# GuixingLin/akka-allreduce

Measured on AMD Instinct MI355X. Metric: allreduce algbw (GB/s) on 256 MB fp32 buffer at 1/2/4/8 MI355X, higher is better.
Workload: dtype fp32

## Files before the change

### akka_allreduce_amd/_build.py

```python
from __future__ import annotations

import concurrent.futures as cf
import glob
import os
import shlex
import subprocess
import sys
import sysconfig

ROOT = os.path.dirname(os.path.dirname(os.path.abspath(__file__)))
CSRC = os.path.join(ROOT, "csrc")
BUILD = os.path.join(ROOT, "build", "native")
PKG = os.path.join(ROOT, "akka_allreduce_amd")
ROCM = os.environ.get("ROCM_PATH", "/opt/rocm")
ARCH = os.environ.get("AKKA_OFFLOAD_ARCH", "gfx950")

HOST_SOURCES = [
    "engine/host_device.cpp",
    "engine/racecheck.cpp",
    "engine/dataplane.cpp",
    "engine/engine.cpp",
    "transport/sim_p2p.cpp",
    "transport/stream_link.cpp",
    "transport/reactive_link.cpp",
    "transport/rccl_p2p.cpp",
    "transport/ipc_lane.cpp",
    "transport/ipc_p2p.cpp",
    "transport/onesided.cpp",
    "transport/link_probe.cpp",
    "kernels/hip_device.cpp",
    "runtime/watchdog.cpp",
    "bindings/bindings.cpp",
    "bindings/bind_onesided.cpp",
    "bindings/bind_probe.cpp",
]
HIP_SOURCES = [
    "kernels/reduce.hip",
    "kernels/counts.hip",
    "kernels/optim.hip",
    "kernels/pack_bf16.hip",
    "kernels/colsum.hip",
    "kernels/xent.hip",
    "kernels/ipc.hip",
    "kernels/onesided.hip",
    "kernels/probe.hip",
]


def ext_path() -> str:
    return os.path.join(PKG, "_native" + sysconfig.get_config_var("EXT_SUFFIX"))


def _torch_lib() -> str:
    import importlib.util

    spec = importlib.util.find_spec("torch")
    if spec is None or not spec.origin:
        raise RuntimeError("torch is required to locate the HIP runtime / RCCL it ships")
    return os.path.join(os.path.dirname(spec.origin), "lib")


def _headers() -> list[str]:
    return sorted(glob.glob(os.path.join(CSRC, "**", "*.h"), recursive=True))


def _stale(obj: str, src: str, headers: list[str]) -> bool:
    if not os.path.exists(obj):
        return True
    t = os.path.getmtime(obj)
    return os.path.getmtime(src) > t or any(os.path.getmtime(h) > t for h in headers)


def source_hash(root: str | None = None) -> str | None:
    import hashlib

    csrc = os.path.join(root or ROOT, "csrc")
    files = [os.path.join(csrc, r) for r in HOST_SOURCES + HIP_SOURCES]
    files += sorted(glob.glob(os.path.join(csrc, "**", "*.h"), recursive=True))
    if not all(os.path.exists(f) for f in files[: len(HOST_SOURCES) + len(HIP_SOURCES)]):
        return None
    h = hashlib.sha256(ARCH.encode())
    for f in files:
        if not os.path.exists(f):
            continue
        h.update(os.path.relpath(f, csrc).encode() + b"\0")
        with open(f, "rb") as fh:
            h.update(fh.read())
        h.update(b"\0")
    return h.hexdigest()


def hash_path(ext: str | None = None) -> str:
    return (ext or ext_path()) + ".srchash"


def stale_reason(ext: str | None = None, root: str | None = None) -> str | None:
    ext = ext or ext_path()
    if not os.path.exists(ext):
        return "not built"
    want = source_hash(root)
    if want is None:
        return None
    try:
        with open(hash_path(ext)) as f:
            have = f.read().strip()
    except OSError:
        return "no source hash recorded next to the module"
    return None if have == want else "sources changed since the module was built"


def have_compiler() -> bool:
    import shutil

    return os.path.exists(os.path.join(ROCM, "bin", "hipcc")) and shutil.which("g++") is not None


def _run(cmd: list[str], verbose: bool) -> None:
    if verbose:
        print(" ".join(shlex.quote(c) for c in cmd), flush=True)
    r = subprocess.run(cmd, stdout=subprocess.PIPE, stderr=subprocess.STDOUT, text=True)
    if r.returncode != 0:
        raise RuntimeError(f"build step failed ({r.returncode}):\n{' '.join(cmd)}\n{r.stdout}")


def build(force: bool = False, jobs: int | None = None, verbose: bool = False, sanitize: str | None = None) -> str:
    import fcntl

    tag = sanitize.replace(",", "-") if sanitize else None
    bdir = os.path.join(ROOT, "build", f"native-{tag}") if tag else BUILD
    os.makedirs(bdir, exist_ok=True)
    with open(os.path.join(bdir, ".lock"), "w") as lk:
        fcntl.flock(lk, fcntl.LOCK_EX)
        try:
            return _build_locked(bdir, tag, force, jobs, verbose, sanitize)
        finally:
            fcntl.flock(lk, fcntl.LOCK_UN)


def _build_locked(bdir: str, tag, force: bool, jobs, verbose: bool, sanitize) -> str:
    import pybind11

    out = os.path.join(bdir, "_native" + sysconfig.get_config_var("EXT_SUFFIX")) if tag else ext_path()
    digest = source_hash()
    py_inc = sysconfig.get_paths()["include"]
    opt = ["-O1", "-g", "-fno-omit-frame-pointer", f"-fsanitize={sanitize}"] if sanitize else ["-O3"]
    common = ["-fPIC", "-std=c++17", "-Wall", "-Wno-unused-function", "-I" + CSRC]
    host_flags = opt + common + [
        "-D__HIP_PLATFORM_AMD__",
        "-I" + os.path.join(ROCM, "include"),
        "-I" + pybind11.get_include(),
        "-I" + py_inc,
        "-fvisibility=hidden",
    ]
    hip_flags = ["-O3"] + common + [f"--offload-arch={ARCH}", "-I" + os.path.join(ROCM, "include")]
    headers = _headers()

    def plan(everything: bool):
        steps, objs = [], []
        for rel in HOST_SOURCES + HIP_SOURCES:
            src = os.path.join(CSRC, rel)
            obj = os.path.join(bdir, rel.replace("/", "_") + ".o")
            objs.append(obj)
            if everything or _stale(obj, src, headers):
                cc = [os.path.join(ROCM, "bin", "hipcc"), *hip_flags] if rel.endswith(".hip") else ["g++", *host_flags]
                steps.append([*cc, "-c", src, "-o", obj])
        return steps, objs

    steps, objs = plan(force)
    mismatch = os.path.exists(out) and stale_reason(out) is not None
    if mismatch and not steps:
        steps, objs = plan(True)
    jobs = jobs or min(8, os.cpu_count() or 4)
    with cf.ThreadPoolExecutor(max_workers=jobs) as ex:
        for f in [ex.submit(_run, s, verbose) for s in steps]:
            f.result()
    if force or steps or not os.path.exists(out) or mismatch:
        tlib = _torch_lib()
        linker = ["g++", f"-fsanitize={sanitize}"] if sanitize else [os.path.join(ROCM, "bin", "hipcc")]
        link = [
            *linker,
            "-shared",
            "-fPIC",
            *objs,
            "-o",
            out + ".tmp",
            "-L" + tlib,
            "-lamdhip64",
            "-lrccl",
            f"-Wl,-rpath,{tlib}",
        ]
        _run(link, verbose)
        os.replace(out + ".tmp", out)
        if digest is not None:
            with open(hash_path(out) + ".tmp", "w") as f:
                f.write(digest + "\n")
            os.replace(hash_path(out) + ".tmp", hash_path(out))
    return out


if __name__ == "__main__":
    san = next((a.split("=", 1)[1] for a in sys.argv if a.startswith("--sanitize=")), None)
    path = build(force="--force" in sys.argv, verbose="-v" in sys.argv, sanitize=san)
    print(path)
```

### akka_allreduce_amd/models/mlp.py

```python
from __future__ import annotations

from typing import Optional

import torch
import torch.nn as nn
import torch.nn.functional as F

from ..ops.colsum import colsum
from ..ops.xent import cross_entropy
from ..parallel.dp import AllreduceFn, GradientBucket


def _mm_into(a: torch.Tensor, b: torch.Tensor, out: torch.Tensor) -> None:
    if a.dtype == out.dtype:
        torch.mm(a, b, out=out)
        return
    try:
        torch.mm(a, b, out_dtype=out.dtype, out=out)
    except (TypeError, RuntimeError):
        out.copy_(torch.mm(a, b))


class _LinearIntoBucket(torch.autograd.Function):

    @staticmethod
    def forward(ctx, x, w, b, gw, gb, ws=None, bs=None):
        dt = torch.get_autocast_dtype(x.device.type) if torch.is_autocast_enabled(x.device.type) else None
        with torch.autocast(device_type=x.device.type, enabled=False):
            if dt is not None and ws is not None and bs is not None and ws.dtype == dt and bs.dtype == dt:
                xc, wc, bc = x.to(dt), ws, bs
            elif dt is not None:
                xc, wc, bc = x.to(dt), w.to(dt), b.to(dt)
            else:
                xc, wc, bc = x, w, b
            y = F.linear(xc, wc, bc)
        ctx.save_for_backward(xc, wc)
        ctx.gw, ctx.gb = gw, gb
        return y

    @staticmethod
    def backward(ctx, go):
        xc, wc = ctx.saved_tensors
        go2 = go.reshape(-1, go.shape[-1]).to(wc.dtype)
        _mm_into(go2.t(), xc.reshape(-1, xc.shape[-1]), ctx.gw)
        if go2.is_cuda and go2.dtype == torch.bfloat16 and ctx.gb.dtype == torch.float32 and ctx.gb.is_contiguous():
            colsum(go2, out=ctx.gb.view(-1))
        else:
            torch.sum(go2, 0, dtype=ctx.gb.dtype, out=ctx.gb)
        gx = (go2 @ wc).reshape(*go.shape[:-1], wc.shape[1]) if ctx.needs_input_grad[0] else None
        return gx, None, None, None, None, None, None


class _LinearReluIntoBucket(torch.autograd.Function):

    @staticmethod
    def forward(ctx, x, w, b, gw, gb, ws, bs):
        dt = torch.get_autocast_dtype(x.device.type)
        with torch.autocast(device_type=x.device.type, enabled=False):
            xc = x.to(dt)
            wc = ws if ws is not None else w.to(dt)
            bc = bs if bs is not None else b.to(dt)
            x2 = xc.reshape(-1, xc.shape[-1])
            h = torch._addmm_activation(bc, x2, wc.t(), use_gelu=False)
        ctx.save_for_backward(x2, wc, h)
        ctx.gw, ctx.gb, ctx.xshape = gw, gb, xc.shape
        return h.reshape(*xc.shape[:-1], wc.shape[0])

    @staticmethod
    def backward(ctx, go):
        x2, wc, h = ctx.saved_tensors
        go2 = go.reshape(-1, go.shape[-1]).to(wc.dtype).contiguous()
        g = torch.empty_like(go2)
        colsum(go2, out=ctx.gb.view(-1), relu_of=h, masked_out=g)
        _mm_into(g.t(), x2, ctx.gw)
        gx = (g @ wc).reshape(ctx.xshape) if ctx.needs_input_grad[0] else None
        return gx, None, None, None, None, None, None


class MLP(nn.Module):
    def __init__(self, d_in: int, d_hidden: int, d_out: int):
        super().__init__()
        self.fc1 = nn.Linear(d_in, d_hidden)
        self.fc2 = nn.Linear(d_hidden, d_out)
        self.direct_grads = False
        self.last_step_direct = False
        self.shadow_bucket: Optional[GradientBucket] = None

    def _linear(self, fc: nn.Linear, x: torch.Tensor) -> torch.Tensor:
        if self.direct_grads and torch.is_grad_enabled():
            sb = self.shadow_bucket
            ws = sb.shadow_of(fc.weight) if sb is not None else None
            bs = sb.shadow_of(fc.bias) if sb is not None else None
            return _LinearIntoBucket.apply(x, fc.weight, fc.bias, fc.weight.grad, fc.bias.grad, ws, bs)
        return fc(x)

    def _linear_relu(self, fc: nn.Linear, x: torch.Tensor) -> torch.Tensor:
        if (self.direct_grads and torch.is_grad_enabled() and x.is_cuda and torch.is_autocast_enabled("cuda")
                and torch.get_autocast_dtype("cuda") == torch.bfloat16 and fc.bias is not None
                and fc.bias.grad is not None and fc.bias.grad.is_contiguous()):
            sb = self.shadow_bucket
            ws = sb.shadow_of(fc.weight) if sb is not None else None
            bs = sb.shadow_of(fc.bias) if sb is not None else None
            return _LinearReluIntoBucket.apply(x, fc.weight, fc.bias, fc.weight.grad, fc.bias.grad, ws, bs)
        return F.relu(self._linear(fc, x))

    def forward(self, x: torch.Tensor) -> torch.Tensor:
        return self._linear(self.fc2, self._linear_relu(self.fc1, x))


def dp_sgd_step(model: nn.Module, x: torch.Tensor, y: torch.Tensor, lr: float,
                allreduce: Optional[AllreduceFn], bucket: Optional[GradientBucket] = None,
                sync_loss: bool = True, compute_dtype: Optional[torch.dtype] = None,
                direct_grads: bool = True, shadow_weights: bool = True, fused_loss: bool = True,
                optimizer=None):
    if optimizer is not None:
        if bucket is not None and optimizer.bucket is not bucket:
            raise ValueError("dp_sgd_step: the optimizer was built on another bucket")
        bucket = optimizer.bucket
    if bucket is None:
        bucket = getattr(model, "_akka_bucket", None)
        if bucket is None:
            bucket = GradientBucket(list(model.parameters()))
            model._akka_bucket = bucket
    loss = _forward_backward(model, x, y, bucket, compute_dtype, direct_grads, shadow_weights, fused_loss)
    bucket.update_from(allreduce, lr, optimizer or bucket.sgd)
    return float(loss.detach()) if sync_loss else loss.detach()


def _forward_backward(model: nn.Module, x: torch.Tensor, y: torch.Tensor, bucket: GradientBucket,
                      compute_dtype: Optional[torch.dtype], direct_grads: bool, shadow_weights: bool,
                      fused_loss: bool, grad_seed: Optional[torch.Tensor] = None) -> torch.Tensor:
    bucket.rebind()
    direct = isinstance(model, MLP) and direct_grads and bucket.bound() \
        and set(map(id, model.parameters())) == set(map(id, bucket.params))
    try:
        if direct:
            model.direct_grads = True
            lowp = compute_dtype if (shadow_weights and compute_dtype is not None
                                     and compute_dtype != torch.float32) else None
            model.shadow_bucket = bucket if bucket.use_shadow(lowp) else None
        else:
            bucket.use_shadow(None)
            bucket.zero_()
        if compute_dtype is not None and compute_dtype != torch.float32:
            with torch.autocast(device_type=x.device.type, dtype=compute_dtype):
                logits = model(x)
            loss = cross_entropy(logits, y) if fused_loss else F.cross_entropy(logits.float(), y)
        else:
            loss = F.cross_entropy(model(x), y)
        loss.backward(grad_seed)
    finally:
        if isinstance(model, MLP):
            model.direct_grads = False
            model.shadow_bucket = None
            model.last_step_direct = direct
    return loss


class GraphedDPStep:

    def __init__(self, model: "MLP", bucket: GradientBucket, x: torch.Tensor, y: torch.Tensor,
                 compute_dtype: Optional[torch.dtype] = None, shadow_weights: bool = True, warmup: int = 3,
                 allreduce: Optional[AllreduceFn] = None, lr: Optional[float] = None, optimizer=None):
        if not (x.is_cuda and isinstance(model, MLP)):
            raise ValueError("GraphedDPStep: an MLP on a GPU")
        if optimizer is not None and optimizer.bucket is not bucket:
            raise ValueError("GraphedDPStep: the optimizer was built on another bucket")
        if bucket.pflat is None or not bucket.bound() or not bucket.params_bound():
            raise ValueError("GraphedDPStep: needs GradientBucket(flatten_params=True) bound to the model")
        self.model, self.bucket, self.rule = model, bucket, optimizer or bucket.sgd
        self.compute_dtype = compute_dtype
        self.lowp = compute_dtype if (shadow_weights and compute_dtype is not None
                                      and compute_dtype != torch.float32) else None
        lowx = compute_dtype if (compute_dtype is not None and compute_dtype != torch.float32
                                 and x.is_floating_point() and x.dtype == torch.float32) else None
        self.sx = x.detach().to(lowx) if lowx is not None else x.detach().clone()
        self.sy = y.detach().clone()
        self._seed = torch.ones((), dtype=torch.float32, device=x.device)
        self._ptrs = self._pointers()

        self.allreduce = allreduce if (allreduce is not None and getattr(allreduce, "capturable", False)) else None
        if allreduce is not None and self.allreduce is None:
            raise ValueError("GraphedDPStep: this allreduce keeps host-side round state; pass it at call time")
        if self.allreduce is not None and lr is None:
            raise ValueError("GraphedDPStep: a captured update needs its learning rate")
        self.lr = lr
        self._out = torch.empty_like(bucket.wire if bucket.wire is not None else bucket.flat) \
            if self.allreduce is not None else None
        self.replays = 0

        def fb():
            loss = _forward_backward(model, self.sx, self.sy, bucket, compute_dtype, True, shadow_weights, True,
                                     grad_seed=self._seed)
            if self.allreduce is not None:
                bucket.update_from(self.allreduce, float(lr), self.rule, out_buf=self._out)
            return loss

        side = torch.cuda.Stream(device=x.device)
        side.wait_stream(torch.cuda.current_stream(x.device))
        snap = (bucket.snapshot(), [s.clone() for s in self.rule.state_tensors()]) \
            if self.allreduce is not None else None
        with torch.cuda.stream(side):
            for _ in range(warmup):
                fb()
        side.synchronize()
        self._side = side
        self.graph = torch.cuda.CUDAGraph()
        with torch.cuda.graph(self.graph, stream=side):
            self.loss = fb().detach()
        torch.cuda.current_stream(x.device).wait_stream(side)
        if snap is not None:
            bucket.restore(snap[0])
            for s, keep in zip(self.rule.state_tensors(), snap[1]):
                s.copy_(keep)
            if self._device_lr():
                self.rule.set_lr(float(lr))
        self._ptrs = self._pointers()

    def static_inputs(self):
        return self.sx, self.sy

    def _pointers(self):
        return self.bucket.pointers(), self.rule.state_pointers()

    def _device_lr(self) -> bool:
        return bool(getattr(self.rule, "device_lr", False))

    def __call__(self, x: torch.Tensor, y: torch.Tensor, lr: float, allreduce: Optional[AllreduceFn],
                 sync_loss: bool = False):
        b = self.bucket
        if self._pointers() != self._ptrs:
            raise RuntimeError("GraphedDPStep: a parameter, gradient, shadow, wire, residual or optimizer state "
                               "buffer moved since the capture")
        if b.use_shadow(self.lowp) != (self.lowp is not None and b.sflat is not None):
            raise RuntimeError("GraphedDPStep: the bf16 shadow is no longer usable")
        if x.data_ptr() != self.sx.data_ptr():
            self.sx.copy_(x)
        if y.data_ptr() != self.sy.data_ptr():
            self.sy.copy_(y)
        if self.allreduce is not None:
            if allreduce is not None and allreduce is not self.allreduce:
                raise RuntimeError("GraphedDPStep: the step captured another allreduce")
            if self._device_lr():
                if lr != self.rule.lr:
                    self.rule.set_lr(lr)
                self.lr = lr
            elif lr != self.lr:
                raise RuntimeError(f"GraphedDPStep: the update was captured with lr={self.lr}")
            self.graph.replay()
            self.replays += 1
            self.allreduce.note_replays(1)
            b.shadow_written()
        else:
            self.graph.replay()
            b.update_from(allreduce, lr, self.rule)
        return float(self.loss) if sync_loss else self.loss


def synthetic_batch(batch: int, d_in: int, n_classes: int, *, device, generator: Optional[torch.Generator] = None):
    x = torch.randn(batch, d_in, device=device, generator=generator)
    w = torch.arange(d_in * n_classes, device=device, dtype=torch.float32).reshape(d_in, n_classes).sin()
    y = (x @ w).argmax(dim=1)
    return x, y
```

### akka_allreduce_amd/ops/__init__.py

```python
from .colsum import colsum
from .compress import pack_bf16
from .reduce import chunk_reduce, count_expand
from .xent import cross_entropy

__all__ = ["chunk_reduce", "colsum", "count_expand", "cross_entropy", "pack_bf16"]
```

### csrc/bindings/bindings.cpp

```cpp
#include <hip/hip_runtime.h>
#include <pybind11/functional.h>
#include <pybind11/pybind11.h>
#include <pybind11/stl.h>

#include <algorithm>
#include <chrono>
#include <condition_variable>
#include <cstdlib>
#include <cstring>
#include <deque>
#include <map>
#include <mutex>
#include <set>

#include "../engine/engine.h"
#include "../kernels/kernels.h"
#include "../runtime/frames.h"
#include "../runtime/watchdog.h"
#include "../transport/ipc_p2p.h"
#include "../transport/p2p.h"
#include "../transport/reactive_link.h"
#include "harness_p2p.h"
#include "../transport/stream_link.h"

// ... 715 lines not shown
      .def(py::init([](int32_t n) { return PyLoopbackHub{std::make_shared<LoopbackHub>(n)}; }))
      .def("bytes_moved", [](const PyLoopbackHub& h) { return h.hub->bytes; });

  py::class_<PyPairHub>(m, "PairLoopbackHub")
      .def(py::init([](int32_t n) { return PyPairHub{std::make_shared<PairHub>(n)}; }))
      .def("bytes_moved", [](const PyPairHub& h) {
        std::lock_guard<std::mutex> lk(h.hub->mu);
        return h.hub->bytes;
      })
      .def("release_all", [](const PyPairHub& h) {
        std::lock_guard<std::mutex> lk(h.hub->mu);
        for (auto* f : h.hub->flags) __atomic_store_n(f, 0x7fffffffu, __ATOMIC_SEQ_CST);
      });

  py::class_<PySimHub>(m, "SimHub")
      .def(py::init([](int32_t n, bool collectives) { return PySimHub{make_sim_hub(n, collectives)}; }),
           py::arg("n"), py::arg("collectives") = false)
      .def("bytes_moved", [](const PySimHub& h) { return sim_bytes_moved(h.hub); });

  py::class_<WorkerCore>(m, "WorkerCore")
      .def(py::init<py::object, std::string, int32_t, std::string, bool, int32_t>(), py::arg("host"),
           py::arg("link") = "outbox", py::arg("device") = -1, py::arg("dtype") = "float32",
           py::arg("deferred") = false, py::arg("lag") = 2)
      .def("init", &WorkerCore::init)
      .def("connect_rccl", &WorkerCore::connect_rccl, py::arg("uid"), py::arg("rank"), py::arg("nranks"),
           py::arg("members") = std::vector<int32_t>{})
      .def("rebuild_transport", &WorkerCore::rebuild_transport)
      .def("connect_sim", &WorkerCore::connect_sim)
      .def("connect_rccl_shape", &WorkerCore::connect_rccl_shape)
      .def("connect_local", &WorkerCore::connect_local)
      .def("connect_callback", &WorkerCore::connect_callback)
      .def("connect_loopback", &WorkerCore::connect_loopback)
      .def("connect_loopback_pair", &WorkerCore::connect_loopback_pair)
      .def("connect_async_callback", &WorkerCore::connect_async_callback)
      .def("attach", &WorkerCore::attach)
      .def("start", &WorkerCore::start)
      .def("poll", &WorkerCore::poll)
      .def("in_flight", &WorkerCore::in_flight)
      .def("wait_activity", &WorkerCore::wait_activity)
      .def("reactive", &WorkerCore::reactive)
      .def("scatter_in", &WorkerCore::scatter_in)
      .def("reduce_in", &WorkerCore::reduce_in)
      .def("peer_terminated", &WorkerCore::peer_terminated)
      .def("fast_round", &WorkerCore::fast_round)
      .def("bind_input", &WorkerCore::bind_input)
      .def("bind_output", &WorkerCore::bind_output, py::arg("round"), py::arg("out"), py::arg("counts"),
           py::arg("stream") = 0, py::arg("has_stream") = false)
      .def("unbind", &WorkerCore::unbind)
      .def("models_streams", &WorkerCore::models_streams)
      .def("create_stream", &WorkerCore::create_stream)
      .def("declare_access", &WorkerCore::declare_access)
      .def("race_reports", &WorkerCore::race_reports)
      .def("race_count", &WorkerCore::race_count)
      .def("sync_stream", &WorkerCore::sync_stream)
      .def("stream_wait_done", &WorkerCore::stream_wait_done)
      .def("sync_done", &WorkerCore::sync_done)
      .def("exec_on_producer", &WorkerCore::exec_on_producer)
      .def("sync_all", &WorkerCore::sync_all)
      .def("expand_counts", &WorkerCore::expand_counts)
      .def("drain", &WorkerCore::drain)
      .def("drain_frames", &WorkerCore::drain_frames)
      .def("apply_frame", &WorkerCore::apply_frame)
      .def("streams", &WorkerCore::streams)
      .def("state", &WorkerCore::state)
      .def("p2p_info", &WorkerCore::p2p_info)
      .def("p2p_check", &WorkerCore::p2p_check)
      .def("set_lane", &WorkerCore::set_lane)
      .def("set_graphs", &WorkerCore::set_graphs)
      .def("set_exact_unit_bytes", &WorkerCore::set_exact_unit_bytes)
      .def("connect_none", &WorkerCore::connect_none)
      .def("connect_ipc_p2p", &WorkerCore::connect_ipc_p2p)
      .def("adopt_transport", &WorkerCore::adopt_transport)
      .def("connect_adopted", &WorkerCore::connect_adopted)
      .def("transport_id", &WorkerCore::transport_id)
      .def("p2p_handle", &WorkerCore::p2p_handle)
      .def("p2p_open", &WorkerCore::p2p_open)
      .def("ipc_handle", &WorkerCore::ipc_handle, py::arg("capacity") = 0, py::arg("share") = nullptr)
      .def("ipc_open", &WorkerCore::ipc_open)
      .def("ipc_error", &WorkerCore::ipc_error)
      .def("ipc_close", &WorkerCore::ipc_close)
      .def("ipc_round_direct", &WorkerCore::ipc_round_direct, py::arg("in_ptr"), py::arg("out_ptr"), py::arg("stream"),
           py::arg("counts") = 0, py::arg("n") = 0, py::arg("finish") = false)
      .def("ipc_error_now", &WorkerCore::ipc_error_now)
      .def("ipc_device_rounds", &WorkerCore::ipc_device_rounds)
      .def("ipc_current_round", &WorkerCore::ipc_current_round)
      .def("ipc_set_mode", &WorkerCore::ipc_set_mode, py::arg("mode"), py::arg("fused") = false,
           py::arg("threads") = 0, py::arg("lite") = -1)
      .def("scatter_count", &WorkerCore::scatter_count)
      .def("reduced_arrivals", &WorkerCore::reduced_arrivals);

  m.def("sim_step", [](const PySimHub& hub, std::vector<WorkerCore*> cores, uint32_t rotate) {
    std::vector<Device*> devs;
    for (auto* c : cores) devs.push_back(c->device());
    return sim_step(hub.hub, devs, rotate);
  }, py::arg("hub"), py::arg("cores"), py::arg("rotate") = 0);
  m.def("sim_run", [](const PySimHub& hub, std::vector<WorkerCore*> cores, int64_t max_iters) {
    std::vector<Device*> devs;
    for (auto* c : cores) devs.push_back(c->device());
    sim_run(hub.hub, devs, max_iters);
  }, py::arg("hub"), py::arg("cores"), py::arg("max_iters") = 100000000);

  m.def("rccl_unique_id", []() {
    auto v = rccl_unique_id();
    return py::bytes(reinterpret_cast<const char*>(v.data()), v.size());
  });
  m.def("rccl_version", []() { return std::string(rccl_version_string()); });
  m.def("watchdog_arm", &watchdog_arm, py::arg("seconds"), py::arg("line"), py::arg("to_stdout"),
        py::arg("debug_path") = "", py::arg("exit_code") = 3, py::arg("tail_bytes") = 4096,
        py::arg("beacon_path") = "",
        "Native phase watchdog (runtime/watchdog.h): on expiry write `line` and _exit(exit_code)");
  m.def("watchdog_disarm", &watchdog_disarm);
  m.def("watchdog_set_out_fd", &watchdog_set_out_fd);
  m.def("watchdog_install_sigterm", &watchdog_install_sigterm);
  m.def("watchdog_track_child", &watchdog_track_child, py::arg("pid"));
  m.def("watchdog_untrack_child", &watchdog_untrack_child, py::arg("pid"));
  m.def("json_escape", &json_escape);
  m.def("hw_queue_probe", [](int32_t kmax, int32_t wait_ms) {
    py::gil_scoped_release nogil;
    uint32_t* flag = nullptr;
    if (hipHostMalloc(reinterpret_cast<void**>(&flag), 64, hipHostMallocCoherent) != hipSuccess)
      throw AkkaError("probe: hipHostMalloc failed");
    *flag = 0;
    void* buf = nullptr;
    if (hipMalloc(&buf, 1 << 20) != hipSuccess) throw AkkaError("probe: hipMalloc failed");
    std::vector<hipStream_t> parked;
    int32_t result = kmax + 1;
    for (int32_t k = 1; k <= kmax; ++k) {
      hipStream_t s;
      hipStreamCreateWithFlags(&s, hipStreamNonBlocking);
      hipStreamWaitValue32(s, flag, 1, hipStreamWaitValueGte, 0xFFFFFFFFu);
      parked.push_back(s);
      hipStream_t f;
      hipStreamCreateWithFlags(&f, hipStreamNonBlocking);
      hipEvent_t e;
      hipEventCreateWithFlags(&e, hipEventDisableTiming);
      hipMemsetAsync(buf, k & 0xff, 1 << 20, f);
      hipEventRecord(e, f);
      auto t0 = std::chrono::steady_clock::now();
      bool done = false;
      while (std::chrono::steady_clock::now() - t0 < std::chrono::milliseconds(wait_ms)) {
        if (hipEventQuery(e) == hipSuccess) {
          done = true;
          break;
        }
      }
      if (!done) {
        result = k;
        __atomic_store_n(flag, 1u, __ATOMIC_SEQ_CST);
        hipEventSynchronize(e);
      }
      hipEventDestroy(e);
      parked.push_back(f);
      if (!done) break;
    }
    __atomic_store_n(flag, 1u, __ATOMIC_SEQ_CST);
    for (auto s : parked) {
      hipStreamSynchronize(s);
      hipStreamDestroy(s);
    }
    hipFree(buf);
    hipHostFree(flag);
    return result;
  }, py::arg("kmax") = 40, py::arg("wait_ms") = 200);
  m.def("tournament", [](int32_t n) {
    std::vector<std::vector<int32_t>> rounds;
    for (int32_t t = 0; t < tournament_rounds(n); ++t) {
      std::vector<int32_t> partner(static_cast<size_t>(n), 0);
      for (int32_t x = 0; x < n; ++x) partner[size_t(x)] = tournament_partner(n, t, x);
      rounds.push_back(partner);
    }
    return rounds;
  }, "partner[x] per ncclCommSplit round of the pair-communicator setup (>= n: sits out)");

  py::class_<P2P>(m, "P2PEndpoint")
      .def("rank", &P2P::rank)
      .def("nranks", &P2P::nranks)
      .def("info", [](const P2P& p) {
        P2PInfo i = p.info();
        py::dict d;
        d["kind"] = i.kind;
        d["nranks"] = i.nranks;
        d["rank"] = i.rank;
        d["device"] = i.device;
        d["comms"] = i.comms;
        return d;
      })
      .def("check", &P2P::check)
      .def("has_collectives", &P2P::has_collectives)
      .def("rebuild", [](P2P& p, py::bytes uid, std::vector<int32_t> members) {
        std::string s = uid;
        return p.rebuild(std::vector<uint8_t>(s.begin(), s.end()), members);
      })
      .def("reduce_scatter", [](P2P& p, uintptr_t stream, uintptr_t send, uintptr_t recv, size_t count,
                                const std::string& dtype) {
        p.reduce_scatter(reinterpret_cast<StreamH>(stream), reinterpret_cast<const void*>(send),
                         reinterpret_cast<void*>(recv), count, dtype == "bfloat16" ? DType::BF16 : DType::F32);
      })
      .def("all_gather", [](P2P& p, uintptr_t stream, uintptr_t send, uintptr_t recv, size_t count,
                            const std::string& dtype) {
        p.all_gather(reinterpret_cast<StreamH>(stream), reinterpret_cast<const void*>(send),
                     reinterpret_cast<void*>(recv), count, dtype == "bfloat16" ? DType::BF16 : DType::F32);
      })
      .def("group", [](P2P& p, uintptr_t stream, const std::vector<std::tuple<bool, int32_t, uintptr_t, size_t>>& ops) {
        std::vector<P2POp> v;
        v.reserve(ops.size());
        for (const auto& o : ops)
          v.push_back({std::get<0>(o), std::get<1>(o), reinterpret_cast<void*>(std::get<2>(o)), std::get<3>(o)});
        p.group(reinterpret_cast<StreamH>(stream), v);
      });
  m.def("rccl_endpoint", [](py::bytes uid, int32_t rank, int32_t nranks, int32_t device, bool pairs,
                            std::vector<int32_t> members) {
    std::string s = uid;
    std::vector<uint8_t> v(s.begin(), s.end());
    return pairs ? make_rccl_pair_p2p(v, rank, nranks, device) : make_rccl_p2p(v, rank, nranks, device, members);
  }, py::arg("uid"), py::arg("rank"), py::arg("nranks"), py::arg("device"), py::arg("pairs") = false,
     py::arg("members") = std::vector<int32_t>{});

  m.def("reduce", [](uintptr_t dst, std::vector<uintptr_t> srcs, int64_t n, std::string dtype, uintptr_t stream,
                     std::string impl) {
    const DType dt = parse_dtype(dtype);
    ReduceImpl im = reduce_impl_from_name(impl.c_str());
    std::vector<const void*> ptrs;
    for (auto p : srcs) ptrs.push_back(reinterpret_cast<const void*>(p));
    AKKA_CHECK(!ptrs.empty(), "reduce: no sources");
    for (const auto& spec : split_reduce(reinterpret_cast<void*>(dst), ptrs, n)) launch_reduce(as_stream(stream), spec, dt, im);
  }, py::arg("dst"), py::arg("srcs"), py::arg("n"), py::arg("dtype") = "float32", py::arg("stream") = 0,
        py::arg("impl") = "auto");
  m.def("count_expand", [](uintptr_t out, const CountsArgs& table, uintptr_t stream) {
    launch_count_expand(as_stream(stream), reinterpret_cast<int32_t*>(out), counts_table(table));
  });
  m.def("count_mean", [](uintptr_t dst, uintptr_t src, const CountsArgs& table, const std::string& dtype,
                         uintptr_t stream, bool axpy, float alpha, uintptr_t shadow, const std::string& src_dtype) {
    const DType dt = parse_dtype(dtype);
    launch_count_mean(as_stream(stream), reinterpret_cast<void*>(dst), reinterpret_cast<const void*>(src),
                      counts_table(table), dt, src_dtype.empty() ? dt : parse_dtype(src_dtype), axpy, alpha,
                      reinterpret_cast<void*>(shadow));
  }, py::arg("dst"), py::arg("src"), py::arg("table"), py::arg("dtype"), py::arg("stream"), py::arg("axpy") = false,
     py::arg("alpha") = 0.f, py::arg("shadow") = 0, py::arg("src_dtype") = "");
  m.def("count_optim", [](const std::string& kind, uintptr_t p, uintptr_t mom, uintptr_t v, uintptr_t shadow,
                          uintptr_t src, const std::string& src_dtype, const CountsArgs& table, uintptr_t t,
                          uintptr_t sq, uintptr_t stream, bool nt, double lr, double weight_decay, double momentum,
                          bool nesterov, double beta1, double beta2, double eps, double max_norm) {
    AKKA_CHECK(kind == "sgd" || kind == "adamw", "count_optim: kind is 'sgd' or 'adamw'");
    const OptimSpec o{kind == "adamw" ? OptimKind::AdamW : OptimKind::SGD, lr, weight_decay, momentum, nesterov,
                      beta1, beta2, eps, max_norm};
    launch_count_optim(as_stream(stream), reinterpret_cast<float*>(p), reinterpret_cast<float*>(mom),
                       reinterpret_cast<float*>(v), reinterpret_cast<void*>(shadow),
                       reinterpret_cast<const void*>(src), parse_dtype(src_dtype), counts_table(table), o,
                       reinterpret_cast<const int32_t*>(t), reinterpret_cast<const float*>(sq), nt);
  }, py::arg("kind"), py::arg("p"), py::arg("m"), py::arg("v"), py::arg("shadow"), py::arg("src"),
     py::arg("src_dtype"), py::arg("table"), py::arg("t"), py::arg("sq"), py::arg("stream") = 0,
     py::arg("nt") = false, py::kw_only(), py::arg("lr"), py::arg("weight_decay") = 0.0, py::arg("momentum") = 0.0,
     py::arg("nesterov") = false, py::arg("beta1") = 0.9, py::arg("beta2") = 0.999, py::arg("eps") = 1e-8,
     py::arg("max_norm") = 0.0);
  m.def("count_optim_groups", [](const std::string& kind, uintptr_t p, uintptr_t mom, uintptr_t v, uintptr_t shadow,
                                 uintptr_t src, const std::string& src_dtype, const CountsArgs& table, uintptr_t t,
                                 uintptr_t sq, uintptr_t seg_end, uintptr_t seg_group, uintptr_t rows,
                                 const std::vector<int64_t>& host_seg_end, const std::vector<int32_t>& host_seg_group,
                                 int32_t ngroups, uintptr_t stream, double momentum, bool nesterov, double beta1,
                                 double beta2, double eps, double max_norm) {
    AKKA_CHECK(kind == "sgd" || kind == "adamw", "count_optim_groups: kind is 'sgd' or 'adamw'");
    AKKA_CHECK(!host_seg_end.empty() && host_seg_end.size() == host_seg_group.size(),
               "count_optim_groups: one group per segment");
    const OptimSpec o{kind == "adamw" ? OptimKind::AdamW : OptimKind::SGD, 0.0, 0.0, momentum, nesterov,
                      beta1, beta2, eps, max_norm};
    OptimGroups g;
    g.seg_end = reinterpret_cast<const int64_t*>(seg_end);
    g.seg_group = reinterpret_cast<const int32_t*>(seg_group);
    g.rows = reinterpret_cast<const float*>(rows);
    g.nseg = int32_t(host_seg_end.size());
    g.ngroups = ngroups;
    g.host_seg_end = host_seg_end.data();
    g.host_seg_group = host_seg_group.data();
    launch_count_optim_groups(as_stream(stream), reinterpret_cast<float*>(p), reinterpret_cast<float*>(mom),
                              reinterpret_cast<float*>(v), reinterpret_cast<void*>(shadow),
                              reinterpret_cast<const void*>(src), parse_dtype(src_dtype), counts_table(table), o, g,
                              reinterpret_cast<const int32_t*>(t), reinterpret_cast<const float*>(sq));
  }, py::arg("kind"), py::arg("p"), py::arg("m"), py::arg("v"), py::arg("shadow"), py::arg("src"),
     py::arg("src_dtype"), py::arg("table"), py::arg("t"), py::arg("sq"), py::arg("seg_end"), py::arg("seg_group"),
     py::arg("rows"), py::arg("host_seg_end"), py::arg("host_seg_group"), py::arg("ngroups"), py::arg("stream") = 0,
     py::kw_only(), py::arg("momentum") = 0.0, py::arg("nesterov") = false, py::arg("beta1") = 0.9,
     py::arg("beta2") = 0.999, py::arg("eps") = 1e-8, py::arg("max_norm") = 0.0);
  m.def("count_sqnorm", [](uintptr_t sq, uintptr_t src, const std::string& src_dtype, const CountsArgs& table,
                           uintptr_t part, uintptr_t ticket, uintptr_t stream) {
    launch_count_sqnorm(as_stream(stream), reinterpret_cast<float*>(sq), reinterpret_cast<const void*>(src),
                        parse_dtype(src_dtype), counts_table(table), reinterpret_cast<float*>(part),
                        reinterpret_cast<uint32_t*>(ticket));
  }, py::arg("sq"), py::arg("src"), py::arg("src_dtype"), py::arg("table"), py::arg("part"), py::arg("ticket"),
     py::arg("stream") = 0);
  m.def("count_sqnorm_partials", &count_sqnorm_partials);
  m.def("pack_bf16", [](uintptr_t dst, uintptr_t src, uintptr_t residual, int64_t n, uintptr_t stream) {
    AKKA_CHECK(n >= 0 && (n == 0 || (dst != 0 && src != 0)), "pack_bf16: null buffer");
    launch_pack_bf16(as_stream(stream), reinterpret_cast<void*>(dst), reinterpret_cast<const float*>(src),
                     reinterpret_cast<float*>(residual), n);
  }, py::arg("dst"), py::arg("src"), py::arg("residual"), py::arg("n"), py::arg("stream") = 0);
  m.def("colsum_bf16", [](uintptr_t out, uintptr_t in, int64_t M, int64_t ncol, uintptr_t part, uintptr_t tickets,
                          int32_t splits, uintptr_t stream, bool lite, uintptr_t act, uintptr_t gout) {
    launch_colsum_bf16(as_stream(stream), reinterpret_cast<float*>(out), reinterpret_cast<const void*>(in), M, ncol,
                       reinterpret_cast<float*>(part), reinterpret_cast<uint32_t*>(tickets), splits, lite,
                       reinterpret_cast<const void*>(act), reinterpret_cast<void*>(gout));
  }, py::arg("out"), py::arg("in"), py::arg("M"), py::arg("ncol"), py::arg("part"), py::arg("tickets"),
     py::arg("splits"), py::arg("stream"), py::arg("lite") = true, py::arg("act") = 0, py::arg("gout") = 0);
  m.def("colsum_row_splits", &colsum_row_splits);
  m.def("xent_fwd", [](uintptr_t x, uintptr_t y, int64_t B, int64_t C, uintptr_t lse, uintptr_t rowloss, uintptr_t out,
                       uintptr_t ticket, uintptr_t stream) {
    launch_xent_fwd(as_stream(stream), reinterpret_cast<const void*>(x), reinterpret_cast<const int64_t*>(y), B, C,
                    reinterpret_cast<float*>(lse), reinterpret_cast<float*>(rowloss), reinterpret_cast<float*>(out),
                    reinterpret_cast<uint32_t*>(ticket));
  });
  m.def("xent_bwd", [](uintptr_t x, uintptr_t y, int64_t B, int64_t C, uintptr_t lse, uintptr_t stat, uintptr_t go,
                       uintptr_t gx, uintptr_t stream) {
    launch_xent_bwd(as_stream(stream), reinterpret_cast<const void*>(x), reinterpret_cast<const int64_t*>(y), B, C,
                    reinterpret_cast<const float*>(lse), reinterpret_cast<const float*>(stat),
                    reinterpret_cast<const float*>(go), reinterpret_cast<void*>(gx));
  });
  m.def("geometry", [](int64_t S, int32_t N, int64_t C) {
    Geometry g(S, N, C);
    py::dict d;
    std::vector<std::pair<int64_t, int64_t>> blocks;
    std::vector<int32_t> nch;
    for (int32_t j = 0; j < N; ++j) {
      blocks.push_back({g.block_start(j), g.block_end(j)});
      nch.push_back(g.num_chunks(j));
    }
    d["step"] = g.step;
    d["blocks"] = blocks;
    d["num_chunks"] = nch;
    d["total_chunks"] = g.total_chunks();
    return d;
  });
  m.def("float_threshold", &float_threshold);
  m.def("ipc_p2p_plan", [](std::vector<std::tuple<bool, int32_t, int64_t, int32_t>> ops, int32_t nranks,
                           int64_t piece, std::vector<uint32_t> dead, std::vector<uint32_t> send_seq,
                           std::vector<uint32_t> recv_seq) {
    std::vector<P2POp> v;
    for (auto& t : ops) v.push_back({std::get<0>(t), std::get<1>(t), nullptr, size_t(std::get<2>(t)), std::get<3>(t)});
    dead.resize(size_t(nranks), 0);
    IpcP2PPlan plan = plan_ipc_p2p_group(v, nranks, piece, 2, dead.data(), send_seq, recv_seq);
    py::list queues;
    for (size_t q = 0; q + 1 < plan.qstart.size(); ++q) {
      py::list ql;
      for (int32_t i = plan.qstart[q]; i < plan.qstart[q + 1]; ++i) {
        const IpcP2POp& o = plan.ops[size_t(i)];
        ql.append(py::make_tuple(bool(o.send), int(o.peer), int(o.ch), o.bytes, o.seq));
      }
      queues.append(ql);
    }
    return py::make_tuple(queues, send_seq, recv_seq, plan.bytes_sent);
  });
  m.def("ipc_layout", [](int32_t N, int32_t np, int32_t nslots, int32_t wpp) {
    py::dict d;
    std::vector<int64_t> lane, p2p;
    for (int32_t src = 0; src < N; ++src)
      for (int32_t j = 0; j < np; ++j) lane.push_back(ipc_flag_push(src, j, np));
    for (int32_t j = 0; j < np; ++j)
      for (int32_t part = 0; part < kIpcReduceSplit; ++part) lane.push_back(ipc_flag_reduced(j, part, N, np));
    for (int32_t src = 0; src < N; ++src)
      for (int32_t j = 0; j < np; ++j)
        for (int32_t part = 0; part < kIpcReduceSplit; ++part) lane.push_back(ipc_flag_gather(src, j, part, N, np));
    lane.push_back(ipc_flag_error(N, np));
    for (int32_t r = 0; r < N; ++r)
      for (int32_t ch = 0; ch < 2; ++ch)
        for (int32_t sl = 0; sl < nslots; ++sl)
          for (int32_t w = 0; w < wpp; ++w) {
            p2p.push_back(ipc_p2p_flag_written(r, ch, sl, w, 2, nslots, wpp));
            p2p.push_back(ipc_p2p_flag_consumed(r, ch, sl, w, N, 2, nslots, wpp));
          }
    d["lane_flags"] = lane;
    d["lane_flag_bytes"] = int64_t(ipc_flag_bytes(N, np));
    d["p2p_flags"] = p2p;
    d["p2p_flag_bytes"] = int64_t(ipc_p2p_flag_bytes(N, 2, nslots, wpp));
    d["stride"] = kIpcFlagStride;
    d["window_slots"] = ipc_window_slots(N);
    return d;
  });
  m.attr("build_arch") = "gfx950";
}
```

### csrc/kernels/kernels.h

```cpp
#pragma once

#include <hip/hip_runtime.h>

#include "../engine/device.h"

namespace akka {

enum class ReduceImpl : int32_t {
  Auto = 0,
  Vec = 1,
  Lds = 2,
  Scalar = 3,
  VecNts = 4,
  VecNtl = 5,
  VecBoth = 6,
};
ReduceImpl reduce_impl_from_name(const char* name);

void launch_reduce(hipStream_t s, const ReduceSpec& spec, DType dt, ReduceImpl impl);
struct CountsTable {
  const int32_t* counts;
  int64_t S, step;
  int32_t N;
  int64_t C;
  int32_t kmax;
  int64_t regions() const { return int64_t(N) * kmax; }
  void check(const char* who) const {
    AKKA_CHECK(regions() > 0 && step >= 0 && C > 0, std::string(who) + ": bad geometry");
  }
};
void launch_count_expand(hipStream_t s, int32_t* out, const CountsTable& t);
void launch_count_mean(hipStream_t s, void* dst, const void* src, const CountsTable& t, DType dt, DType src_dt,
                       bool axpy = false, float alpha = 0.f, void* shadow = nullptr);
enum class OptimKind : int32_t { SGD = 0, AdamW = 1 };
struct OptimSpec {
  OptimKind kind = OptimKind::SGD;
  double lr = 0, weight_decay = 0;
  double momentum = 0;
  bool nesterov = false;
  double beta1 = 0.9, beta2 = 0.999, eps = 1e-8;
  double max_norm = 0;
};
void launch_count_optim(hipStream_t s, float* p, float* m, float* v, void* shadow, const void* src, DType src_dt,
                        const CountsTable& ct, const OptimSpec& o, const int32_t* t, const float* sq, bool nt = false);
struct OptimGroups {
  const int64_t* seg_end = nullptr;
  const int32_t* seg_group = nullptr;
  const float* rows = nullptr;
  int32_t nseg = 0, ngroups = 0;
  const int64_t* host_seg_end = nullptr;
  const int32_t* host_seg_group = nullptr;
};
void launch_count_optim_groups(hipStream_t s, float* p, float* m, float* v, void* shadow, const void* src,
                               DType src_dt, const CountsTable& ct, const OptimSpec& o, const OptimGroups& g,
                               const int32_t* t, const float* sq);
void launch_count_sqnorm(hipStream_t s, float* sq, const void* src, DType src_dt, const CountsTable& ct, float* part,
                         uint32_t* ticket);
int32_t count_sqnorm_partials();
void launch_pack_bf16(hipStream_t s, void* q, const float* g, float* r, int64_t n);
void launch_colsum_bf16(hipStream_t s, float* out, const void* in, int64_t M, int64_t ncol, float* part,
                        uint32_t* tickets, int32_t splits, bool lite = true, const void* act = nullptr,
                        void* gout = nullptr);
int32_t colsum_row_splits(int64_t M, int64_t ncol);
void launch_xent_fwd(hipStream_t s, const void* x, const int64_t* y, int64_t B, int64_t C, float* lse,
                     float* rowloss, float* out, uint32_t* ticket);
void launch_xent_bwd(hipStream_t s, const void* x, const int64_t* y, int64_t B, int64_t C, const float* lse,
                     const float* stat, const float* go, void* gx);
void launch_poison_counts(hipStream_t s, const uint32_t* flag, int32_t* counts, int64_t n);
void launch_fill_counts(hipStream_t s, const uint32_t* flag, int32_t* counts, int32_t value, int64_t n);
ReduceImpl reduce_impl_from_env();
const char* reduce_impl_name(ReduceImpl i);

}
```

Before: 3555.

## Add custom bf16 MFMA weight-gradient kernel writing fp32 directly into gradient bucket

Adds a HIP kernel that computes the weight gradient g^T x from bf16 inputs with 32x32x16 MFMA instructions and LDS staging, storing fp32 results straight into the output. The MLP matmul helper routes bf16-by-bf16-to-fp32 products through it by default, replacing the library mixed-dtype GEMM. This targets the library's overhead for small-K, large-output shapes. It risks being slower than a tuned library GEMM and does not touch the allreduce path that the metric measures.

```diff
diff --git a/akka_allreduce_amd/_build.py b/akka_allreduce_amd/_build.py
--- a/akka_allreduce_amd/_build.py
+++ b/akka_allreduce_amd/_build.py
@@ -40,6 +40,7 @@
     "kernels/optim.hip",
     "kernels/pack_bf16.hip",
     "kernels/colsum.hip",
+    "kernels/wgrad.hip",
     "kernels/xent.hip",
     "kernels/ipc.hip",
     "kernels/onesided.hip",
diff --git a/akka_allreduce_amd/models/mlp.py b/akka_allreduce_amd/models/mlp.py
--- a/akka_allreduce_amd/models/mlp.py
+++ b/akka_allreduce_amd/models/mlp.py
@@ -1,5 +1,6 @@
 from __future__ import annotations
 
+import os
 from typing import Optional
 
 import torch
@@ -7,13 +8,33 @@
 import torch.nn.functional as F
 
 from ..ops.colsum import colsum
+from ..ops.wgrad import wgrad
 from ..ops.xent import cross_entropy
 from ..parallel.dp import AllreduceFn, GradientBucket
+
+
+_WGRAD = os.environ.get("AKKA_WGRAD", "1") != "0"
+_WGRAD_LIBRARY_SHAPES: frozenset = frozenset()
+
+
+def _on_gpu(*ts: torch.Tensor) -> bool:
+    return all(t.is_cuda for t in ts)
+
+
+def _wgrad_takes(a: torch.Tensor, b: torch.Tensor, out: torch.Tensor) -> bool:
+    return (_WGRAD and a.dim() == 2 and b.dim() == 2 and out.dim() == 2
+            and a.dtype == torch.bfloat16 and b.dtype == torch.bfloat16 and out.dtype == torch.float32
+            and _on_gpu(a, b, out) and a.t().is_contiguous() and b.is_contiguous() and out.stride(-1) == 1
+            and a.numel() > 0 and b.numel() > 0
+            and (a.shape[1], a.shape[0], b.shape[1]) not in _WGRAD_LIBRARY_SHAPES)
 
 
 def _mm_into(a: torch.Tensor, b: torch.Tensor, out: torch.Tensor) -> None:
     if a.dtype == out.dtype:
         torch.mm(a, b, out=out)
+        return
+    if _wgrad_takes(a, b, out):
+        wgrad(a.t(), b, out)
         return
     try:
         torch.mm(a, b, out_dtype=out.dtype, out=out)
diff --git a/akka_allreduce_amd/ops/__init__.py b/akka_allreduce_amd/ops/__init__.py
--- a/akka_allreduce_amd/ops/__init__.py
+++ b/akka_allreduce_amd/ops/__init__.py
@@ -1,6 +1,7 @@
 from .colsum import colsum
 from .compress import pack_bf16
 from .reduce import chunk_reduce, count_expand
+from .wgrad import wgrad
 from .xent import cross_entropy
 
-__all__ = ["chunk_reduce", "colsum", "count_expand", "cross_entropy", "pack_bf16"]
+__all__ = ["chunk_reduce", "colsum", "count_expand", "cross_entropy", "pack_bf16", "wgrad"]
diff --git a/akka_allreduce_amd/ops/wgrad.py b/akka_allreduce_amd/ops/wgrad.py
--- /dev/null
+++ b/akka_allreduce_amd/ops/wgrad.py
@@ -0,0 +1,41 @@
+from __future__ import annotations
+
+import os
+
+import torch
+
+from .._native_loader import load as _load
+
+_NT = os.environ.get("AKKA_WGRAD_NT", "0") == "1"
+
+
+def _rows(t: torch.Tensor) -> bool:
+    return t.dim() == 2 and (t.stride(1) == 1 or t.shape[1] == 1) and (t.stride(0) >= t.shape[1] or t.shape[0] == 1)
+
+
+def _ld(t: torch.Tensor) -> int:
+    return t.stride(0) if t.shape[0] > 1 else max(t.stride(0), t.shape[1])
+
+
+def native_ok(g: torch.Tensor, x: torch.Tensor, out: torch.Tensor) -> bool:
+    return (g.is_cuda and x.is_cuda and out.is_cuda and g.device == x.device == out.device
+            and g.dtype == torch.bfloat16 and x.dtype == torch.bfloat16 and out.dtype == torch.float32
+            and _rows(g) and _rows(x) and _rows(out) and min(g.shape[0], g.shape[1], x.shape[1]) >= 1)
+
+
+def wgrad(g: torch.Tensor, x: torch.Tensor, out: torch.Tensor, nt: bool | None = None) -> torch.Tensor:
+    if g.dim() != 2 or x.dim() != 2 or out.dim() != 2:
+        raise ValueError("wgrad expects 2-D tensors")
+    K, M = g.shape
+    if x.shape[0] != K or tuple(out.shape) != (M, x.shape[1]):
+        raise ValueError(f"wgrad: g {tuple(g.shape)}, x {tuple(x.shape)} and out {tuple(out.shape)} do not match")
+    if not native_ok(g, x, out):
+        if g.dtype == out.dtype and x.dtype == out.dtype:
+            torch.mm(g.t(), x, out=out)
+        else:
+            out.copy_(torch.mm(g.t().to(out.dtype), x.to(out.dtype)))
+        return out
+    n = _load()
+    n.wgrad_bf16(out.data_ptr(), _ld(out), g.data_ptr(), _ld(g), x.data_ptr(), _ld(x), K, M,
+                 x.shape[1], torch.cuda.current_stream(g.device).cuda_stream, _NT if nt is None else bool(nt))
+    return out
diff --git a/csrc/bindings/bindings.cpp b/csrc/bindings/bindings.cpp
--- a/csrc/bindings/bindings.cpp
+++ b/csrc/bindings/bindings.cpp
@@ -1041,6 +1041,12 @@
   }, py::arg("out"), py::arg("in"), py::arg("M"), py::arg("ncol"), py::arg("part"), py::arg("tickets"),
      py::arg("splits"), py::arg("stream"), py::arg("lite") = true, py::arg("act") = 0, py::arg("gout") = 0);
   m.def("colsum_row_splits", &colsum_row_splits);
+  m.def("wgrad_bf16", [](uintptr_t out, int64_t ldo, uintptr_t g, int64_t ldg, uintptr_t x, int64_t ldx, int64_t K,
+                         int64_t M, int64_t N, uintptr_t stream, bool nt) {
+    launch_wgrad_bf16(as_stream(stream), reinterpret_cast<float*>(out), ldo, reinterpret_cast<const void*>(g), ldg,
+                      reinterpret_cast<const void*>(x), ldx, K, M, N, nt);
+  }, py::arg("out"), py::arg("ldo"), py::arg("g"), py::arg("ldg"), py::arg("x"), py::arg("ldx"), py::arg("K"),
+     py::arg("M"), py::arg("N"), py::arg("stream"), py::arg("nt") = false);
   m.def("xent_fwd", [](uintptr_t x, uintptr_t y, int64_t B, int64_t C, uintptr_t lse, uintptr_t rowloss, uintptr_t out,
                        uintptr_t ticket, uintptr_t stream) {
     launch_xent_fwd(as_stream(stream), reinterpret_cast<const void*>(x), reinterpret_cast<const int64_t*>(y), B, C,
diff --git a/csrc/kernels/kernels.h b/csrc/kernels/kernels.h
--- a/csrc/kernels/kernels.h
+++ b/csrc/kernels/kernels.h
@@ -62,6 +62,8 @@
                         uint32_t* tickets, int32_t splits, bool lite = true, const void* act = nullptr,
                         void* gout = nullptr);
 int32_t colsum_row_splits(int64_t M, int64_t ncol);
+void launch_wgrad_bf16(hipStream_t s, float* out, int64_t ldo, const void* G, int64_t ldg, const void* X, int64_t ldx,
+                       int64_t K, int64_t M, int64_t N, bool nt = false);
 void launch_xent_fwd(hipStream_t s, const void* x, const int64_t* y, int64_t B, int64_t C, float* lse,
                      float* rowloss, float* out, uint32_t* ticket);
 void launch_xent_bwd(hipStream_t s, const void* x, const int64_t* y, int64_t B, int64_t C, const float* lse,
diff --git a/csrc/kernels/wgrad.hip b/csrc/kernels/wgrad.hip
--- /dev/null
+++ b/csrc/kernels/wgrad.hip
@@ -0,0 +1,145 @@
+#include <hip/hip_runtime.h>
+
+#include "elem.h"
+#include "kernels.h"
+#include "launch_util.h"
+
+namespace akka {
+
+namespace {
+
+using bf16x8 = __bf16 __attribute__((ext_vector_type(8)));
+using f32x16 = float __attribute__((ext_vector_type(16)));
+
+template <bool VEC>
+__device__ __forceinline__ v4u wg_load8(const bf16_t* __restrict__ src, int64_t ld, int k, int K, int64_t r0,
+                                        int64_t R) {
+  v4u v = {0u, 0u, 0u, 0u};
+  if (k >= K) return v;
+  const bf16_t* p = src + int64_t(k) * ld + r0;
+  if constexpr (VEC) {
+    if (r0 + 8 <= R) v = *reinterpret_cast<const v4u*>(p);
+  } else {
+#pragma unroll
+    for (int e = 0; e < 8; ++e)
+      if (r0 + e < R) v[e >> 1] |= uint32_t(p[e]) << ((e & 1) * 16);
+  }
+  return v;
+}
+
+constexpr int TM = 128, TN = 128;
+constexpr int KS = 64;
+constexpr int WR = 2, WC = 2;
+constexpr int FM = TM / WR / 32, FN = TN / WC / 32;
+constexpr int kPitch = KS + 8;
+constexpr int kKg = KS / 8;
+constexpr int kNg = kKg * (TM / 8), kNx = kKg * (TN / 8);
+static_assert(WR * WC == kBlock / 64 && FM * 32 * WR == TM && FN * 32 * WC == TN, "waves do not tile the output");
+static_assert(kNg + kNx == kBlock && TM % 16 == 0 && KS % 16 == 0 && (kPitch / 8) % 2 == 1, "staging layout");
+
+template <bool VEC, bool NT>
+__global__ __launch_bounds__(kBlock) __attribute__((amdgpu_waves_per_eu(4, 4))) void wgrad_bf16_kernel(
+    float* __restrict__ out, int64_t ldo, const bf16_t* __restrict__ G, int64_t ldg, const bf16_t* __restrict__ X,
+    int64_t ldx, int K, int M, int N) {
+  __shared__ __attribute__((aligned(16))) bf16_t img[(TM + TN) * kPitch];
+  auto off = [](int row, int kg) { return row * kPitch + ((kg ^ ((row >> 4) & (kKg - 1))) << 3); };
+  const int tid = threadIdx.x, lane = tid & 63, wave = tid >> 6;
+  const int64_t m0 = int64_t(blockIdx.y) * TM, n0 = int64_t(blockIdx.x) * TN;
+
+  const bool isx = tid >= kNg;
+  const int idx = isx ? tid - kNg : tid;
+  const int rg = isx ? idx % (TN / 8) : idx % (TM / 8), kg = isx ? idx / (TN / 8) : idx / (TM / 8);
+  const int srow = (isx ? TM : 0) + rg * 8;
+  const bf16_t* src = isx ? X : G;
+  const int64_t ld = isx ? ldx : ldg, R = isx ? N : M, r0 = (isx ? n0 : m0) + rg * 8;
+
+  const int wm = wave / WC, wn = wave % WC, l31 = lane & 31, half = lane >> 5;
+  f32x16 acc[FM][FN];
+#pragma unroll
+  for (int a = 0; a < FM; ++a)
+#pragma unroll
+    for (int b = 0; b < FN; ++b)
+#pragma unroll
+      for (int q = 0; q < 16; ++q) acc[a][b][q] = 0.f;
+
+  for (int ks = 0; ks < K; ks += KS) {
+    v4u v[8];
+#pragma unroll
+    for (int i = 0; i < 8; ++i) v[i] = wg_load8<VEC>(src, ld, ks + kg * 8 + i, K, r0, R);
+    __syncthreads();
+#pragma unroll
+    for (int r = 0; r < 8; ++r) {
+      v4u w;
+#pragma unroll
+      for (int c = 0; c < 4; ++c) {
+        const uint32_t lo = v[2 * c][r >> 1], hi = v[2 * c + 1][r >> 1];
+        w[c] = (r & 1) ? ((lo >> 16) | (hi & 0xffff0000u)) : ((lo & 0xffffu) | (hi << 16));
+      }
+      *reinterpret_cast<v4u*>(&img[off(srow + r, kg)]) = w;
+    }
+    __syncthreads();
+    const int rem = K - ks;
+    const int steps = rem >= KS ? KS / 16 : (rem + 15) / 16;
+    for (int s = 0; s < steps; ++s) {
+      bf16x8 a[FM], b[FN];
+#pragma unroll
+      for (int t = 0; t < FM; ++t)
+        a[t] = __builtin_bit_cast(
+            bf16x8, *reinterpret_cast<const v4u*>(&img[off((wm * FM + t) * 32 + l31, 2 * s + half)]));
+#pragma unroll
+      for (int t = 0; t < FN; ++t)
+        b[t] = __builtin_bit_cast(
+            bf16x8, *reinterpret_cast<const v4u*>(&img[off(TM + (wn * FN + t) * 32 + l31, 2 * s + half)]));
+#pragma unroll
+      for (int tm = 0; tm < FM; ++tm)
+#pragma unroll
+        for (int tn = 0; tn < FN; ++tn)
+          acc[tm][tn] = __builtin_amdgcn_mfma_f32_32x32x16_bf16(a[tm], b[tn], acc[tm][tn], 0, 0, 0);
+    }
+  }
+
+#pragma unroll
+  for (int tm = 0; tm < FM; ++tm)
+#pragma unroll
+    for (int q = 0; q < 16; ++q) {
+      const int64_t m = m0 + (wm * FM + tm) * 32 + (q & 3) + 8 * (q >> 2) + 4 * half;
+#pragma unroll
+      for (int tn = 0; tn < FN; ++tn) {
+        const int64_t n = n0 + (wn * FN + tn) * 32 + l31;
+        if (m < M && n < N) {
+          float* p = out + m * ldo + n;
+          if constexpr (NT) __builtin_nontemporal_store(acc[tm][tn][q], p);
+          else *p = acc[tm][tn][q];
+        }
+      }
+    }
+}
+
+}
+
+void launch_wgrad_bf16(hipStream_t s, float* out, int64_t ldo, const void* G, int64_t ldg, const void* X, int64_t ldx,
+                       int64_t K, int64_t M, int64_t N, bool nt) {
+  AKKA_CHECK(K >= 1 && M >= 1 && N >= 1, "wgrad: empty shape");
+  AKKA_CHECK(out != nullptr && G != nullptr && X != nullptr, "wgrad: null buffer");
+  AKKA_CHECK(ldo >= N && ldg >= M && ldx >= N, "wgrad: a row stride is shorter than its row");
+  const int64_t tm = (M + TM - 1) / TM, tn = (N + TN - 1) / TN;
+  AKKA_CHECK(K < (int64_t(1) << 31) && N < (int64_t(1) << 31) && tm <= 65535, "wgrad: shape too large");
+  const bool vec = M % 8 == 0 && N % 8 == 0 && ldg % 8 == 0 && ldx % 8 == 0 &&
+                   ((reinterpret_cast<uintptr_t>(G) | reinterpret_cast<uintptr_t>(X)) & 15) == 0;
+  const dim3 grid{uint32_t(tn), uint32_t(tm), 1u};
+#define AKKA_WG(V, T)                                                                                         \
+  hipLaunchKernelGGL((wgrad_bf16_kernel<V, T>), grid, dim3(kBlock), 0, s, out, ldo,                           \
+                     static_cast<const bf16_t*>(G), ldg, static_cast<const bf16_t*>(X), ldx, int(K), int(M), \
+                     int(N))
+  if (vec) {
+    if (nt) AKKA_WG(true, true);
+    else AKKA_WG(true, false);
+  } else {
+    if (nt) AKKA_WG(false, true);
+    else AKKA_WG(false, false);
+  }
+#undef AKKA_WG
+  check_launch("wgrad_bf16");
+}
+
+}
diff --git a/profiles/r10/wgrad/microbench.py b/profiles/r10/wgrad/microbench.py
--- /dev/null
+++ b/profiles/r10/wgrad/microbench.py
@@ -0,0 +1,48 @@
+import json
+import os
+import sys
+
+import torch
+
+sys.path.insert(0, os.path.dirname(os.path.dirname(os.path.dirname(os.path.dirname(os.path.abspath(__file__))))))
+from akka_allreduce_amd.ops.wgrad import wgrad
+
+
+def timeit(f, n=40):
+    for _ in range(5):
+        f()
+    reps = []
+    for _ in range(3):
+        a, b = torch.cuda.Event(enable_timing=True), torch.cuda.Event(enable_timing=True)
+        a.record()
+        for _ in range(n):
+            f()
+        b.record()
+        torch.cuda.synchronize()
+        reps.append(round(a.elapsed_time(b) / n * 1e3, 1))
+    return reps
+
+
+def main():
+    dev = torch.device("cuda", 0)
+    bucket = torch.empty(8192 * 4096 + 8192 + 1000 * 8192 + 1000, device=dev)
+    for (K, M, N, offs) in [(256, 8192, 4096, 0), (256, 1000, 8192, 8192 * 4096 + 8192)]:
+        g = torch.randn(K, M, device=dev).to(torch.bfloat16)
+        x = torch.randn(K, N, device=dev).to(torch.bfloat16)
+        out = bucket[offs:offs + M * N].view(M, N)
+        ref = torch.mm(g.t(), x, out_dtype=torch.float32)
+        r = {"shape": [K, M, N],
+             "lib_us": timeit(lambda: torch.mm(g.t(), x, out_dtype=torch.float32, out=out)),
+             "fill_us": timeit(lambda: out.zero_()), "copy_us": timeit(lambda: out.copy_(ref))}
+        for kk in (1, 64, 128, 192):
+            gk, xk = g[:kk].contiguous(), x[:kk].contiguous()
+            r[f"K{kk}_us"] = timeit(lambda: wgrad(gk, xk, out, nt=False))
+        for nt in (False, True):
+            r["nt_us" if nt else "plain_us"] = timeit(lambda: wgrad(g, x, out, nt=nt))
+        wgrad(g, x, out)
+        r["max_abs_diff_vs_lib"] = float((out - ref).abs().max())
+        print(json.dumps(r), flush=True)
+
+
+if __name__ == "__main__":
+    main()
```

Result: no change. 3552 (-0.1%).
